# yxyxcyx/Real-Time-Recommendation-System-with-Feature-Store

Measured on NVIDIA B200. Metric: top-100 exact-IP QPS over 10M items, higher is better.
Workload: dtype bf16

## Files before the change

real-time-recommendation-system-with-feature-store_b200/csrc/stream_scores.cuh:

```cuda
#pragma once
#include <cstdlib>
#include "host_util.h"
#include "tc_common.cuh"

namespace b200 {

constexpr int ST_EPI_WARP0 = 4;
constexpr int ST_HELP_WARP0 = 12;
constexpr int ST_HELP_WARPS = 4;
constexpr int ST_THREADS = 16 * 32;
constexpr int ST_QTILE_BYTES = 128 * 64 * 2;
constexpr int ST_MAX_STAGES = 16;
constexpr int ST_SMEM_LIMIT = 232448;
constexpr int ST_BAR_BYTES = 512;

struct StreamGeom {
  long long N;
  long long T;
  long long total;
  long long W;
  int Q;
  int KB;
  int S;
  int grid;
// ... 57 lines not shown
__device__ __forceinline__ int geom_first_cta(const StreamGeom& g, int s) { return (int)((s * g.T) / g.W); }
__device__ __forceinline__ int geom_last_cta(const StreamGeom& g, int s) { return (int)(((s + 1) * g.T - 1) / g.W); }


template <int NQ, int BN, class Epi>
__global__ void __launch_bounds__(ST_THREADS, 1)
stream_scores_kernel(const __grid_constant__ CUtensorMap tmap_q, const __grid_constant__ CUtensorMap tmap_x,
                     const StreamGeom g, const typename Epi::Args ea) {
  constexpr int QPT = NQ >= 2 ? NQ / 2 : 1;
  constexpr int EPI_WARPS = NQ >= 2 ? 8 : 4;
  constexpr int STAGE_BYTES = BN * 128;
  static_assert(NQ <= 2, "helper-warp mailboxes are sized for 256 resident rows");
  static_assert(2 * NQ * BN <= 512, "two accumulator buffers must fit the 512 TMEM columns");

  extern __shared__ uint8_t smem_raw[];
  uint8_t* smem = smem_raw + ((1024u - (smem_u32(smem_raw) & 1023u)) & 1023u);
  uint8_t* q_smem = smem;
  uint8_t* ring = smem + NQ * g.KB * ST_QTILE_BYTES;
  uint8_t* tail = ring + g.stages * STAGE_BYTES;
  uint64_t* full_bar = reinterpret_cast<uint64_t*>(tail);
  uint64_t* empty_bar = full_bar + ST_MAX_STAGES;
  uint64_t* acc_full = empty_bar + ST_MAX_STAGES;
  uint64_t* acc_empty = acc_full + 2;
  uint64_t* q_full = acc_empty + 2;
  uint64_t* q_empty = q_full + 1;
  uint32_t* tmem_slot = reinterpret_cast<uint32_t*>(q_empty + 1);
  uint32_t* scratch = reinterpret_cast<uint32_t*>(tail + ST_BAR_BYTES);

  const int warp = threadIdx.x >> 5;
  const int lane = threadIdx.x & 31;

  if (warp == 0 && lane == 0) {
    tma_prefetch_desc(&tmap_q);
    tma_prefetch_desc(&tmap_x);
  }
  if (warp == 1 && lane == 0) {
    for (int s = 0; s < g.stages; ++s) {
      mbar_init(&full_bar[s], 1);
      mbar_init(&empty_bar[s], 1);
    }
    for (int b = 0; b < 2; ++b) {
      mbar_init(&acc_full[b], 1);
      mbar_init(&acc_empty[b], EPI_WARPS);
    }
    mbar_init(q_full, 1);
    mbar_init(q_empty, 1);
    fence_mbar_init();
  }
  if (warp == 2) tmem_alloc(tmem_slot, 512);
  if (warp == 3) Epi::init_scratch(scratch, lane);
  tc_fence_before();
  __syncthreads();
  tc_fence_after();
  const uint32_t tmem_base = *tmem_slot;

  const long long w_begin = (long long)blockIdx.x * g.W;
  long long w_end = w_begin + g.W;
  if (w_end > g.total) w_end = g.total;

  if (warp == 0) {
    {
      const uint64_t pol_q = l2_policy_evict_last();
      uint32_t it = 0, seg = 0;
      for (long long w = w_begin; w < w_end; ++seg) {
        const int s = (int)(w / g.T);
        const long long t0 = w - (long long)s * g.T;
        long long t1 = t0 + (w_end - w);
        if (t1 > g.T) t1 = g.T;
        mbar_wait(q_empty, (seg & 1) ^ 1);
        if (elect_one()) {
          mbar_arrive_expect_tx(q_full, NQ * g.KB * ST_QTILE_BYTES);
          for (int qs = 0; qs < NQ; ++qs)
            for (int kb = 0; kb < g.KB; ++kb)
              tma_load_2d_hint(q_smem + (qs * g.KB + kb) * ST_QTILE_BYTES, &tmap_q, q_full, kb * 64,
                               (s * NQ + qs) * 128, pol_q);
        }
        __syncwarp();
        for (long long t = t0; t < t1; ++t) {
          for (int kb = 0; kb < g.KB; ++kb, ++it) {
            const int st = it % g.stages;
            const uint32_t ph = (it / g.stages) & 1;
            mbar_wait(&empty_bar[st], ph ^ 1);
            if (elect_one()) {
              mbar_arrive_expect_tx(&full_bar[st], STAGE_BYTES);
              tma_load_2d(ring + st * STAGE_BYTES, &tmap_x, &full_bar[st], kb * 64, (int)(t * BN));
            }
            __syncwarp();
          }
        }
        w += t1 - t0;
      }
    }
  } else if (warp == 1) {
    {
      const uint32_t idesc = umma_idesc_bf16(128, BN);
      const uint64_t desc_base = umma_desc_k_sw128(0);
      const uint32_t q_lo = (smem_u32(q_smem) & 0x3FFFFu) >> 4;
      const uint32_t ring_lo = (smem_u32(ring) & 0x3FFFFu) >> 4;
      uint32_t it = 0, seg = 0, tc = 0;
      for (long long w = w_begin; w < w_end; ++seg) {
        const int s = (int)(w / g.T);
        const long long t0 = w - (long long)s * g.T;
        long long t1 = t0 + (w_end - w);
        if (t1 > g.T) t1 = g.T;
        mbar_wait(q_full, seg & 1);
        tc_fence_after();
        for (long long t = t0; t < t1; ++t, ++tc) {
          const uint32_t buf = tc & 1;
          mbar_wait(&acc_empty[buf], ((tc >> 1) & 1) ^ 1);
          tc_fence_after();
          for (int kb = 0; kb < g.KB; ++kb, ++it) {
            const int st = it % g.stages;
            const uint32_t ph = (it / g.stages) & 1;
            mbar_wait(&full_bar[st], ph);
            tc_fence_after();
            if (elect_one()) {
              const uint64_t b_desc = desc_base + (ring_lo + ((st * STAGE_BYTES) >> 4));
#pragma unroll
              for (int qs = 0; qs < NQ; ++qs) {
                const uint64_t a_desc = desc_base + (q_lo + (((qs * g.KB + kb) * ST_QTILE_BYTES) >> 4));
                const uint32_t d_addr = tmem_base + (buf * NQ + qs) * BN;
#pragma unroll
                for (int k = 0; k < 4; ++k) umma_bf16(d_addr, a_desc + 2 * k, b_desc + 2 * k, idesc, (kb | k) != 0);
              }
              umma_commit(&empty_bar[st]);
              if (kb == g.KB - 1) umma_commit(&acc_full[buf]);
            }
            __syncwarp();
          }
        }
        if (elect_one()) umma_commit(q_empty);
        __syncwarp();
        w += t1 - t0;
      }
    }
  } else if (warp >= ST_EPI_WARP0 && warp < ST_EPI_WARP0 + EPI_WARPS) {
    const int ew = warp - ST_EPI_WARP0;
    const int quarter = warp & 3;
    const int half = ew >> 2;
    Epi epi;
    uint32_t tc = 0;
    for (long long w = w_begin; w < w_end;) {
      const int s = (int)(w / g.T);
      const long long t0 = w - (long long)s * g.T;
      long long t1 = t0 + (w_end - w);
      if (t1 > g.T) t1 = g.T;
      const int part = (int)blockIdx.x - geom_first_cta(g, s);
      int qslot[QPT];
      long long qrow[QPT];
#pragma unroll
      for (int a = 0; a < QPT; ++a) {
        qslot[a] = (half * QPT + a) * 128 + quarter * 32 + lane;
        const long long q = (long long)s * (128 * NQ) + qslot[a];
        qrow[a] = q < g.Q ? q : -1;
      }
      epi.template begin_segment<128 * NQ, QPT>(ea, g, s, part, qrow, qslot, lane, scratch);
      for (long long t = t0; t < t1; ++t, ++tc) {
        const uint32_t buf = tc & 1;
        epi.template pre_tile<BN, QPT>(ea, g, qslot, lane, scratch);
        mbar_wait(&acc_full[buf], (tc >> 1) & 1);
        tc_fence_after();
#pragma unroll
        for (int a = 0; a < QPT; ++a) {
          const uint32_t taddr =
              tmem_base + (static_cast<uint32_t>(quarter * 32) << 16) + (buf * NQ + half * QPT + a) * BN;
          epi.template tile<BN>(ea, g, a, taddr, (unsigned long long)t * BN);
        }
        tc_fence_before();
        __syncwarp();
        if (lane == 0) mbar_arrive(&acc_empty[buf]);
      }
      epi.template end_segment<128 * NQ, QPT>(ea, g, s, part, qslot, lane, scratch, (w + (t1 - t0)) >= w_end);
      w += t1 - t0;
    }
    Epi::epilogue_exit(scratch, lane);
  } else if (warp >= ST_HELP_WARP0) {
    Epi::template helper<128 * NQ, EPI_WARPS>(ea, g, warp - ST_HELP_WARP0, lane, scratch);
  }
  tc_fence_before();
  __syncthreads();
  if (warp == 2) {
    tc_fence_after();
    tmem_dealloc(tmem_base, 512);
  }
}

}
```

real-time-recommendation-system-with-feature-store_b200/csrc/stream_scores2.cuh:

```cuda
#pragma once
#include "stream_scores.cuh"

namespace b200 {

__device__ __forceinline__ uint32_t cluster_ctarank() {
  uint32_t r;
  asm volatile("mov.u32 %0, %%cluster_ctarank;" : "=r"(r));
  return r;
}
__device__ __forceinline__ void cluster_sync_all() {
  asm volatile("barrier.cluster.arrive.release.aligned;\n\tbarrier.cluster.wait.acquire.aligned;" ::: "memory");
}
__device__ __forceinline__ uint32_t mapa_u32(uint32_t local, uint32_t rank) {
  uint32_t r;
  asm volatile("mapa.shared::cluster.u32 %0, %1, %2;" : "=r"(r) : "r"(local), "r"(rank));
  return r;
}
__device__ __forceinline__ void mbar_arrive_cluster(uint32_t cluster_addr) {
  asm volatile("mbarrier.arrive.shared::cluster.b64 _, [%0];" ::"r"(cluster_addr) : "memory");
}
__device__ __forceinline__ void tma_load_2d_2sm(void* smem_dst, const CUtensorMap* m, uint32_t bar_cluster_addr, int c0,
                                                int c1) {
  asm volatile(
      "cp.async.bulk.tensor.2d.cta_group::2.shared::cluster.global.mbarrier::complete_tx::bytes [%0], [%1, {%3, %4}], [%2];"
// ... 125 lines not shown
stream_scores2_kernel(const __grid_constant__ CUtensorMap tmap_q, const __grid_constant__ CUtensorMap tmap_x,
                      const StreamGeom g, const typename Epi::Args ea) {
  constexpr int EPI_WARPS = 8;
  constexpr int S2_ROWS = S2Shape<NQ2>::ROWS, S2_QUERIES = S2Shape<NQ2>::QUERIES;
  constexpr int S2_STAGE_BYTES = S2Shape<NQ2>::STAGE_BYTES, UMMA_N = S2Shape<NQ2>::UMMA_N;
  constexpr int COLS = 128;
  constexpr int NSUB = NQ2;
  extern __shared__ uint8_t smem_raw[];
  uint8_t* smem = smem_raw + ((1024u - (smem_u32(smem_raw) & 1023u)) & 1023u);
  uint8_t* q_smem = smem;
  uint8_t* ring = smem + NQ2 * g.KB * ST_QTILE_BYTES;
  const int ks = g.ks;
  const int stage_bytes = S2_STAGE_BYTES * ks;
  const int nsteps = g.KB / ks;
  uint8_t* tail = ring + g.stages * stage_bytes;
  uint64_t* full_bar = reinterpret_cast<uint64_t*>(tail);
  uint64_t* empty_bar = full_bar + ST_MAX_STAGES;
  uint64_t* acc_full = empty_bar + ST_MAX_STAGES;
  uint64_t* acc_empty = acc_full + 4;
  uint64_t* q_full = acc_empty + 4;
  uint64_t* q_empty = q_full + 1;
  uint32_t* tmem_slot = reinterpret_cast<uint32_t*>(q_empty + 1);
  uint32_t* scratch = reinterpret_cast<uint32_t*>(tail + ST_BAR_BYTES);

  const int warp = threadIdx.x >> 5;
  const int lane = threadIdx.x & 31;
  const uint32_t rank = cluster_ctarank();
  const bool leader = rank == 0;
  const long long unit = blockIdx.x >> 1;

  if (warp == 0 && lane == 0) {
    tma_prefetch_desc(&tmap_q);
    tma_prefetch_desc(&tmap_x);
  }
  if (warp == 1 && lane == 0) {
    for (int s = 0; s < g.stages; ++s) {
      mbar_init(&full_bar[s], 1);
      mbar_init(&empty_bar[s], 1);
    }
    for (int b = 0; b < 4; ++b) {
      mbar_init(&acc_full[b], 1);
      mbar_init(&acc_empty[b], 2 * EPI_WARPS / NSUB);
    }
    mbar_init(q_full, 1);
    mbar_init(q_empty, 1);
    fence_mbar_init();
  }
  if (warp == 2) tmem_alloc2(tmem_slot, 512);
  if (warp == 3) Epi::init_scratch(scratch, lane);
  tc_fence_before();
  __syncthreads();
  cluster_sync_all();
  tc_fence_after();
  const uint32_t tmem_base = *tmem_slot;

  constexpr bool kDbg = Epi::kDbg;
  const bool dbg_st = kDbg && (g.dbg_stats == 1 || g.dbg_stats == 2 + (int)unit);
  const bool nofeed = kDbg && g.dbg_nofeed != 0;
  const int mma_order = kDbg ? g.mma_order : 0;
  int s;
  long long t0, ntile, tstep;
  bool last_seg;

  if (warp == 0) {
    {
      const uint32_t q_full_leader = mapa_u32(smem_u32(q_full), 0);
      uint32_t it = 0;
      for (int seg = 0; geom2_segment(g, unit, seg, s, t0, ntile, tstep, last_seg); ++seg) {
        mbar_wait(q_empty, (seg & 1) ^ 1);
        if (elect_one()) {
          if (leader) mbar_arrive_expect_tx(q_full, 2 * NQ2 * g.KB * ST_QTILE_BYTES);
          for (int qt = 0; qt < NQ2; ++qt)
            for (int kb = 0; kb < g.KB; ++kb)
              tma_load_2d_2sm(q_smem + (qt * g.KB + kb) * ST_QTILE_BYTES, &tmap_q, q_full_leader, kb * 64,
                              s * S2_QUERIES + qt * 256 + (int)rank * 128);
        }
        __syncwarp();
        if (!nofeed) {
          for (long long ti = 0, t = t0; ti < ntile; ++ti, t += tstep) {
            for (int step = 0; step < nsteps; ++step, ++it) {
              const int st = it % g.stages;
              const uint32_t ph = (it / g.stages) & 1;
              mbar_wait(&empty_bar[st], ph ^ 1);
              if (elect_one()) {
                if (leader) mbar_arrive_expect_tx(&full_bar[st], 2 * stage_bytes);
                const uint32_t bar = mapa_u32(smem_u32(&full_bar[st]), 0);
                for (int a = 0; a < ks; ++a)
                  tma_load_2d_2sm(ring + st * stage_bytes + a * S2_STAGE_BYTES, &tmap_x, bar, (step * ks + a) * 64,
                                  (int)(t * S2_ROWS + rank * (S2_ROWS / 2)));
              }
              __syncwarp();
            }
          }
        }
      }
    }
  } else if (warp == 1) {
    if (leader) {
      const uint32_t idesc = umma_idesc_bf16(256, UMMA_N);
      const uint64_t desc_base = umma_desc_k_sw128(0);
      const uint32_t q_lo = (smem_u32(q_smem) & 0x3FFFFu) >> 4;
      const uint32_t ring_lo = (smem_u32(ring) & 0x3FFFFu) >> 4;
      uint32_t it = 0, tc = 0;
      long long c_acc = 0, c_full = 0;
      for (int seg = 0; geom2_segment(g, unit, seg, s, t0, ntile, tstep, last_seg); ++seg) {
        mbar_wait(q_full, seg & 1);
// ... 44 lines not shown
          tc_fence_after();
          const long long c1 = dbg_st ? clock64() : 0;
          c_acc += c1 - c0;
          for (int step = 0; step < nsteps; ++step, ++it) {
            const int st = it % g.stages;
            const uint32_t ph = (it / g.stages) & 1;
            if (!nofeed) {
              const long long c2 = dbg_st ? clock64() : 0;
              mbar_wait(&full_bar[st], ph);
              tc_fence_after();
              if (dbg_st) c_full += clock64() - c2;
            }
            if (elect_one()) {
              for (int a = 0; a < ks; ++a) {
                const int kb = step * ks + a;
                const uint64_t b_desc = desc_base + (ring_lo + ((st * stage_bytes + a * S2_STAGE_BYTES) >> 4));
                if (mma_order == 3) {
#pragma unroll
                  for (int k = 0; k < 4; ++k) {
#pragma unroll
                    for (int qt = 0; qt < NQ2; ++qt) {
                      const uint64_t a_desc = desc_base + (q_lo + (((qt * g.KB + kb) * ST_QTILE_BYTES) >> 4));
                      umma_bf16_2sm(tmem_base + buf * 256 + qt * 128, a_desc + 2 * k, b_desc + 2 * k, idesc, (kb | k) != 0);
                    }
                  }
                  continue;
                }
#pragma unroll
                for (int qt = 0; qt < NQ2; ++qt) {
                  const uint64_t a_desc = desc_base + (q_lo + (((qt * g.KB + kb) * ST_QTILE_BYTES) >> 4));
                  const uint32_t d_addr = tmem_base + buf * 256 + qt * 128;
#pragma unroll
                  for (int k = 0; k < 4; ++k)
                    umma_bf16_2sm(d_addr, a_desc + 2 * k, b_desc + 2 * k, idesc, (kb | k) != 0);
                }
              }
              if (!nofeed) umma_commit_2sm(&empty_bar[st]);
              if (step == nsteps - 1) {
                for (int sub = 0; sub < NSUB; ++sub) umma_commit_2sm(&acc_full[buf * 2 + sub]);
              }
            }
            __syncwarp();
          }
        }
        if (elect_one()) umma_commit_2sm(q_empty);
        __syncwarp();
      }
      if (dbg_st && lane == 0) {
        atomicAdd(&g_stream_stats[0], (unsigned long long)c_acc);
        atomicAdd(&g_stream_stats[1], (unsigned long long)c_full);
      }
    }
  } else if (warp >= ST_EPI_WARP0 && warp < ST_EPI_WARP0 + EPI_WARPS) {
    const int ew = warp - ST_EPI_WARP0;
    const int quarter = warp & 3;
    const int half = ew >> 2;
    Epi epi;
    uint32_t tc = 0;
    long long c_wait = 0, c_proc = 0;
    const int sub = NSUB == 2 ? half : 0;
    const uint32_t acc_empty_leader[2] = {mapa_u32(smem_u32(&acc_empty[sub]), 0), mapa_u32(smem_u32(&acc_empty[2 + sub]), 0)};
    for (int seg = 0; geom2_segment(g, unit, seg, s, t0, ntile, tstep, last_seg); ++seg) {
      const int part = 0;
      int qslot[1] = {half * 128 + quarter * 32 + lane};
      const long long q = (long long)s * S2_QUERIES + (NQ2 == 2 ? half * 256 : 0) + rank * 128 + quarter * 32 + lane;
      long long qrow[1] = {q < g.Q ? q : -1};
      epi.template begin_segment<S2_SLOTS, 1>(ea, g, s, part, qrow, qslot, lane, scratch);
      for (long long ti = 0, t = t0; ti < ntile; ++ti, t += tstep, ++tc) {
        const uint32_t buf = tc & 1;
        epi.template pre_tile<COLS, 1>(ea, g, qslot, lane, scratch);
        const long long c0 = dbg_st ? clock64() : 0;
        mbar_wait(&acc_full[buf * 2 + sub], (tc >> 1) & 1);
        tc_fence_after();
        const long long c1 = dbg_st ? clock64() : 0;
        const uint32_t taddr = tmem_base + (static_cast<uint32_t>(quarter * 32) << 16) + buf * 256 + half * 128;
        epi.template tile<COLS>(ea, g, 0, taddr, (unsigned long long)t * S2_ROWS + (NQ2 == 1 ? half * 128 : 0));
        tc_fence_before();
        __syncwarp();
        if (lane == 0) mbar_arrive_cluster(acc_empty_leader[buf]);
        if (dbg_st) {
          c_wait += c1 - c0;
          c_proc += clock64() - c1;
        }
      }
      epi.template end_segment<S2_SLOTS, 1>(ea, g, s, part, qslot, lane, scratch, last_seg);
    }
    if (dbg_st && lane == 0) {
      atomicAdd(&g_stream_stats[2], (unsigned long long)c_wait);
      atomicAdd(&g_stream_stats[3], (unsigned long long)c_proc);
      atomicAdd(&g_stream_stats[4], (unsigned long long)tc);
    }
    Epi::epilogue_exit(scratch, lane);
  } else if (warp >= ST_HELP_WARP0) {
    Epi::template helper<S2_SLOTS, EPI_WARPS>(ea, g, warp - ST_HELP_WARP0, lane, scratch);
  }
  tc_fence_before();
  __syncthreads();
  cluster_sync_all();
  if (warp == 2) {
    tc_fence_after();
    tmem_dealloc2(tmem_base, 512);
  }
}

}
```

real-time-recommendation-system-with-feature-store_b200/csrc/tc_common.cuh:

```cuda
#pragma once
#include <cuda.h>
#include <cuda_runtime.h>
#include <cuda_bf16.h>
#include <stdint.h>

namespace b200 {

constexpr uint32_t FULL_MASK = 0xffffffffu;

__device__ __forceinline__ uint32_t smem_u32(const void* p) {
  return static_cast<uint32_t>(__cvta_generic_to_shared(p));
}
__device__ __forceinline__ bool elect_one() {
  uint32_t pred;
  asm volatile(
      "{\n\t.reg .pred p;\n\t"
      "elect.sync _|p, 0xffffffff;\n\t"
      "selp.u32 %0, 1, 0, p;\n\t}\n"
      : "=r"(pred));
  return pred != 0;
}

__device__ __forceinline__ void mbar_init(uint64_t* bar, uint32_t count) {
  asm volatile("mbarrier.init.shared::cta.b64 [%0], %1;" ::"r"(smem_u32(bar)), "r"(count) : "memory");
}
__device__ __forceinline__ void fence_mbar_init() {
  asm volatile("fence.mbarrier_init.release.cluster;" ::: "memory");
}
__device__ __forceinline__ void fence_proxy_async_smem() {
  asm volatile("fence.proxy.async.shared::cta;" ::: "memory");
}
__device__ __forceinline__ void mbar_arrive(uint64_t* bar) {
  asm volatile("mbarrier.arrive.shared::cta.b64 _, [%0];" ::"r"(smem_u32(bar)) : "memory");
}
__device__ __forceinline__ void mbar_arrive_expect_tx(uint64_t* bar, uint32_t bytes) {
  asm volatile("mbarrier.arrive.expect_tx.shared::cta.b64 _, [%0], %1;" ::"r"(smem_u32(bar)), "r"(bytes)
               : "memory");
}
__device__ __forceinline__ bool mbar_try_wait(uint64_t* bar, uint32_t parity) {
  uint32_t ok;
  asm volatile(
      "{\n\t.reg .pred p;\n\t"
      "mbarrier.try_wait.parity.shared::cta.b64 p, [%1], %2;\n\t"
      "selp.u32 %0, 1, 0, p;\n\t}\n"
      : "=r"(ok)
      : "r"(smem_u32(bar)), "r"(parity)
      : "memory");
  return ok != 0;
}
__device__ __forceinline__ void mbar_wait(uint64_t* bar, uint32_t parity) {
  uint32_t spins = 0;
  while (!mbar_try_wait(bar, parity)) {
    if (++spins > (1u << 24)) {
      printf("b200rec: mbarrier wait timed out (block %d thread %d)\n", blockIdx.x, threadIdx.x);
      __trap();
    }
  }
}

__device__ __forceinline__ void tma_prefetch_desc(const CUtensorMap* m) {
  asm volatile("prefetch.tensormap [%0];" ::"l"(reinterpret_cast<uint64_t>(m)) : "memory");
}
__device__ __forceinline__ void tma_load_2d(void* smem_dst, const CUtensorMap* m, uint64_t* bar, int c0, int c1) {
  asm volatile(
      "cp.async.bulk.tensor.2d.shared::cluster.global.mbarrier::complete_tx::bytes [%0], [%1, {%3, %4}], [%2];"
      ::"r"(smem_u32(smem_dst)), "l"(reinterpret_cast<uint64_t>(m)), "r"(smem_u32(bar)), "r"(c0), "r"(c1)
      : "memory");
}
__device__ __forceinline__ void tma_load_2d_hint(void* smem_dst, const CUtensorMap* m, uint64_t* bar, int c0,
                                                  int c1, uint64_t policy) {
  asm volatile(
      "cp.async.bulk.tensor.2d.shared::cluster.global.mbarrier::complete_tx::bytes.L2::cache_hint"
      " [%0], [%1, {%3, %4}], [%2], %5;"
      ::"r"(smem_u32(smem_dst)), "l"(reinterpret_cast<uint64_t>(m)), "r"(smem_u32(bar)), "r"(c0), "r"(c1),
      "l"(policy)
      : "memory");
}
__device__ __forceinline__ uint64_t l2_policy_evict_first() {
  uint64_t p;
  asm volatile("createpolicy.fractional.L2::evict_first.b64 %0, 1.0;" : "=l"(p));
  return p;
// ... 120 lines not shown
```

real-time-recommendation-system-with-feature-store_b200/csrc/topk.cu:

```cuda
#include <cfloat>
#include <cstdlib>
#include <mutex>
#include "stream_scores.cuh"
#include "stream_scores2.cuh"
#include "../../include/b200rec.h"

namespace b200 {

__device__ __forceinline__ int warp_pick_digit(const uint32_t* hist, int& need, int& bucket, int lane) {
  uint32_t c[8];
  uint32_t lane_total = 0;
#pragma unroll
  for (int b = 0; b < 8; ++b) {
    c[b] = hist[lane * 8 + b];
    lane_total += c[b];
  }
  uint32_t incl = lane_total;
#pragma unroll
  for (int o = 1; o < 32; o <<= 1) {
    const uint32_t t = __shfl_down_sync(FULL_MASK, incl, o);
    if (lane + o < 32) incl += t;
  }
  const uint32_t above = incl - lane_total;
  const bool mine = (above < (uint32_t)need) && ((uint32_t)need <= incl);
// ... 520 lines not shown
          __syncwarp();
          if (lane == 0) {
            __threadfence();
            atomicExch(&m->lock, 0u);
            reqs[slot] = 0u;
          }
          __syncwarp();
          if (dbgv(ea) == 2 && lane == 0) atomicAdd(&g_topk_stats[3], (unsigned long long)(clock64() - hb0));
        }
      }
      if (!any) {
        if (finished) break;
        __nanosleep(ea.hsleep);
      }
    }
    if (stamp) {
      unsigned long long ns_end;
      asm volatile("mov.u64 %0, %%globaltimer;" : "=l"(ns_end));
      if (blockIdx.x == 0) g_topk_stats[6] = (unsigned long long)(clock64() - c_begin) * 1000ull / (ns_end - ns_begin + 1);
      atomicMax(&g_topk_stats[5], ~ns_begin);
      atomicMax(&g_topk_stats[7], ns_end);
      if (blockIdx.x < 512) g_cta_end[blockIdx.x] = ns_end;
    }
  }
};

using TopkEpi = TopkEpiT<false>;
using TopkEpiDbg = TopkEpiT<true>;

struct SampleMaxEpi {
  static constexpr bool kDbg = false;
  static constexpr int SCRATCH_BYTES = 64;
  struct Args {
    float* out;
    int ngroups;
    int gw;
  };
  long long qrow[2];

  static __device__ __forceinline__ void init_scratch(uint32_t*, int) {}
  static __device__ __forceinline__ void epilogue_exit(uint32_t*, int) {}
  template <int SLOTS, int EPI_WARPS>
  static __device__ __forceinline__ void helper(const Args&, const StreamGeom&, int, int, uint32_t*) {}

  template <int SLOTS, int QPT>
  __device__ __forceinline__ void begin_segment(const Args&, const StreamGeom&, int, int, const long long (&q)[QPT],
                                                const int (&)[QPT], int, uint32_t*) {
#pragma unroll
    for (int a = 0; a < QPT; ++a) qrow[a] = q[a];
  }
  template <int BN, int QPT>
  __device__ __forceinline__ void pre_tile(const Args&, const StreamGeom&, const int (&)[QPT], int, uint32_t*) {}

  template <int BN>
  __device__ __forceinline__ void tile(const Args& ea, const StreamGeom&, int a, uint32_t taddr,
                                       unsigned long long row0) {
    float run = -INFINITY;
#pragma unroll 1
    for (int c = 0; c < BN; c += 32) {
      uint32_t v[32];
      tmem_ld_32x32(taddr + c, v);
      tmem_ld_wait();
      float m4[4];
#pragma unroll
      for (int j = 0; j < 4; ++j) {
        const float m0 = fmax3(__uint_as_float(v[8 * j + 0]), __uint_as_float(v[8 * j + 1]), __uint_as_float(v[8 * j + 2]));
        const float m1 = fmax3(__uint_as_float(v[8 * j + 3]), __uint_as_float(v[8 * j + 4]), __uint_as_float(v[8 * j + 5]));
        m4[j] = fmax3(m0, m1, fmaxf(__uint_as_float(v[8 * j + 6]), __uint_as_float(v[8 * j + 7])));
      }
      run = fmaxf(run, fmaxf(fmaxf(m4[0], m4[1]), fmaxf(m4[2], m4[3])));
      if (((c + 32) % ea.gw) == 0) {
        if (qrow[a] >= 0) ea.out[(size_t)qrow[a] * ea.ngroups + (row0 + c) / ea.gw] = run;
        run = -INFINITY;
      }
    }
  }

  template <int SLOTS, int QPT>
  __device__ __forceinline__ void end_segment(const Args&, const StreamGeom&, int, int, const int (&)[QPT], int,
                                              uint32_t*, bool) {}
};

constexpr int FIN_THREADS = 256;

template <class Loader>
__device__ void block_select_sort_core(const Loader& load, int n, int k_out, uint64_t* skeys , int P,
                                       uint32_t* hist , int* s_misc ) {
  const int tid = threadIdx.x, lane = tid & 31, warp = tid >> 5;
  if (tid == 0) s_misc[0] = 0;
  __syncthreads();
  int local = 0;
  for (int i = tid; i < n; i += FIN_THREADS) local += load(i) != 0ull;
  for (int o = 16; o > 0; o >>= 1) local += __shfl_xor_sync(FULL_MASK, local, o);
  if (lane == 0 && local) atomicAdd(&s_misc[0], local);
  __syncthreads();
  const int n_valid = s_misc[0];
  uint64_t prefix = 1;
  int shift = 0;
  if (n_valid > k_out) {
    prefix = 0;
    shift = 56;
    int need = k_out;
    for (int pass = 0; pass < 8; ++pass, shift -= 8) {
      hist[tid] = 0;
      __syncthreads();
      for (int i = tid; i < n; i += FIN_THREADS) {
        const uint64_t key = load(i);
        const bool match = (pass == 0) || ((key >> (shift + 8)) == prefix);
        if (match && key != 0ull) atomicAdd(&hist[(uint32_t)(key >> shift) & 255u], 1u);
      }
      __syncthreads();
      if (warp == 0) {
        int bucket;
        const int d = warp_pick_digit(hist, need, bucket, lane);
        if (lane == 0) {
          s_misc[1] = d;
          s_misc[2] = need;
          s_misc[3] = bucket;
        }
      }
      __syncthreads();
      prefix = (prefix << 8) | (uint64_t)s_misc[1];
      need = s_misc[2];
      const int bucket = s_misc[3];
      __syncthreads();
      if (bucket == need) break;
// ... 46 lines not shown

constexpr int FAN_MAX = 16;
struct OutFan {
  int n;
  float* s[FAN_MAX];
  int64_t* i[FAN_MAX];
};

__device__ __forceinline__ void write_result(const uint64_t* skeys, int k_out, int64_t row_offset, float* out_s,
                                             int64_t* out_i) {
  for (int i = threadIdx.x; i < k_out; i += FIN_THREADS) {
    const uint64_t key = skeys[i];
    if (key == 0ull) {
      out_s[i] = -FLT_MAX;
      out_i[i] = -1;
    } else {
      out_s[i] = ord_f32((uint32_t)(key >> 32));
      out_i[i] = (int64_t)(~(uint32_t)key) + row_offset;
    }
  }
}

constexpr int FIN_MAX_SRC = 160;
struct MultiLoader {
  const uint64_t* const* ptr;
  const int* off;
  int nsrc;
  __device__ __forceinline__ uint64_t operator()(int i) const {
    int lo = 0, hi = nsrc - 1;
    while (lo < hi) {
      const int mid = (lo + hi + 1) >> 1;
      if (off[mid] <= i)
        lo = mid;
      else
        hi = mid - 1;
    }
    return __ldcg(ptr[lo] + (i - off[lo]));
  }
};

__global__ void __launch_bounds__(FIN_THREADS)
topk_final_kernel(const StreamGeom g, int v2, int qs , int slots ,
                  const uint64_t* __restrict__ tlists, const QMeta* __restrict__ meta,
                  const uint64_t* __restrict__ lists, const uint32_t* __restrict__ left, int cap, int k, int P,
                  int stage_cap, int64_t row_offset, const OutFan fan) {
  extern __shared__ uint64_t fin_smem[];
  __shared__ uint32_t hist[256];
  __shared__ int s_misc[8];
  __shared__ const uint64_t* s_ptr[FIN_MAX_SRC];
  __shared__ int s_off[FIN_MAX_SRC + 1];
  __shared__ int s_last[FIN_MAX_SRC];
  const int q = blockIdx.x;
  const int s = q / qs, inq = q - s * qs;
  if (v2) {
    for (int u = threadIdx.x; u < g.grid / 2 && u < FIN_MAX_SRC; u += FIN_THREADS) s_last[u] = geom2_last_super(g, u);
    __syncthreads();
  }
  if (threadIdx.x == 0) {
    int n = 0, ns = 0;
    s_ptr[ns] = tlists + (size_t)q * 2 * k + (size_t)meta[q].tsel * k;
    s_off[ns++] = n;
    n += (int)meta[q].tcount;
    const int u0 = v2 ? 0 : geom_first_cta(g, s), u1 = v2 ? g.grid / 2 - 1 : geom_last_cta(g, s);
    for (int u = u0; u <= u1; ++u) {
      if (v2) {
        if (u >= FIN_MAX_SRC || s_last[u] != s) continue;
      } else {
        long long wend = (long long)(u + 1) * g.W;
        if (wend > g.total) wend = g.total;
        if ((int)((wend - 1) / g.T) != s) continue;
      }
      const int cta = v2 ? 2 * u + ((inq >> 7) & 1) : u;
      const int nslot = v2 == 1 ? 2 : 1;
      for (int h = 0; h < nslot && ns < FIN_MAX_SRC; ++h) {
        const int slot = v2 == 1 ? h * 128 + (inq & 127) : (v2 == 2 ? (inq >> 8) * 128 + (inq & 127) : inq);
        const uint32_t l = left[(size_t)cta * slots + slot];
        const int cnt = (int)(l & 0x7FFFFFFFu);
        if (cnt == 0) continue;
        s_ptr[ns] = lists + ((size_t)cta * slots + slot) * (2 * (size_t)cap) + ((l >> 31) ? cap : 0);
        s_off[ns++] = n;
        n += cnt;
      }
    }
    s_off[ns] = n;
    s_misc[5] = ns;
    s_misc[6] = n;
  }
  __syncthreads();
  MultiLoader ld{s_ptr, s_off, s_misc[5]};
  const int n = s_misc[6];
  __syncthreads();
  block_select_sort(ld, n, k, fin_smem, P, hist, s_misc, fin_smem + P, stage_cap);
  for (int d = 0; d < fan.n; ++d)
    write_result(fin_smem, k, row_offset, fan.s[d] + (size_t)q * k, fan.i[d] + (size_t)q * k);
}

struct FloatRowLoader {
  const float* row;
  __device__ __forceinline__ uint64_t operator()(int i) const {
    return (static_cast<uint64_t>(f32_ord(__ldcg(row + i))) << 32) | static_cast<uint64_t>(~(uint32_t)i);
  }
};
__global__ void __launch_bounds__(FIN_THREADS)
sample_topk_kernel(const float* __restrict__ S, int m, int k, int P, int stage_cap, const OutFan fan) {
  extern __shared__ uint64_t fin_smem[];
  __shared__ uint32_t hist[256];
  __shared__ int s_misc[8];
  const int q = blockIdx.x;
  FloatRowLoader ld{S + (size_t)q * m};
  block_select_sort(ld, m, k, fin_smem, P, hist, s_misc, fin_smem + P, stage_cap);
  for (int i = threadIdx.x; i < k; i += FIN_THREADS) {
    const uint64_t key = fin_smem[i];
    const float v = key == 0ull ? -FLT_MAX : ord_f32((uint32_t)(key >> 32));
    for (int d = 0; d < fan.n; ++d) fan.s[d][(size_t)q * k + i] = v;
  }
}

struct PooledLoader {
  const float* vals;
  size_t part_stride;
  int k_in;
  __device__ __forceinline__ uint64_t operator()(int i) const {
    const int p = i / k_in, j = i - p * k_in;
    return (static_cast<uint64_t>(f32_ord(__ldcg(vals + (size_t)p * part_stride + j))) << 32) | static_cast<uint64_t>(~(uint32_t)i);
  }
};
__global__ void __launch_bounds__(FIN_THREADS)
pooled_kth_kernel(const float* __restrict__ vals, int parts, long long Q, int k_in, int k, int P, int stage_cap,
                  float* __restrict__ out_kth) {
  extern __shared__ uint64_t fin_smem[];
  __shared__ uint32_t hist[256];
  __shared__ int s_misc[8];
  const long long q = blockIdx.x;
  PooledLoader ld{vals + (size_t)q * k_in, (size_t)Q * k_in, k_in};
  block_select_sort(ld, parts * k_in, k, fin_smem, P, hist, s_misc, fin_smem + P, stage_cap);
  if (threadIdx.x == 0) {
    const uint64_t key = fin_smem[k - 1];
    out_kth[q] = key == 0ull ? -FLT_MAX : ord_f32((uint32_t)(key >> 32));
  }
}

__global__ void topk_init_from_kernel(QMeta* meta, int Q, const float* __restrict__ tau_init) {
  const int q = blockIdx.x * blockDim.x + threadIdx.x;
  if (q < Q) {
    uint32_t key = f32_ord(tau_init[q]);
    key = key > 64u ? key - 64u : 0u;
    QMeta m;
    m.lock = 0u;
    m.tcount = 0u;
    m.tsel = 0u;
    m.tau = fmaxf(ord_f32(key), nextafterf(-FLT_MAX, 0.f));
    meta[q] = m;
  }
}

__global__ void topk_init_kernel(QMeta* meta, int Q, float tau0) {
  const int q = blockIdx.x * blockDim.x + threadIdx.x;
  if (q < Q) {
    QMeta m;
    m.lock = 0u;
    m.tcount = 0u;
    m.tsel = 0u;
    m.tau = tau0;
    meta[q] = m;
  }
}

struct ListLoader {
  const float* scores;
  const int64_t* ids;
  size_t s_stride, i_stride;
  int k_in;
  __device__ __forceinline__ uint64_t operator()(int i) const {
    const int p = i / k_in, j = i - p * k_in;
    const int64_t id = ids[(size_t)p * i_stride + j];
    return id < 0 ? 0ull : make_key(scores[(size_t)p * s_stride + j], (uint32_t)id);
  }
};

__global__ void __launch_bounds__(FIN_THREADS)
topk_merge_kernel(const float* __restrict__ scores, const int64_t* __restrict__ ids, int parts, long long Q, int k_in,
                  int k_out, int P, int stage_cap, long long s_stride, long long i_stride,
                  float* __restrict__ out_scores, int64_t* __restrict__ out_ids) {
  extern __shared__ uint64_t fin_smem[];
  __shared__ uint32_t hist[256];
  __shared__ int s_misc[8];
  const long long q = blockIdx.x;
  ListLoader ld;
  ld.scores = scores + (size_t)q * k_in;
  ld.ids = ids + (size_t)q * k_in;
  ld.s_stride = (size_t)s_stride;
  ld.i_stride = (size_t)i_stride;
  ld.k_in = k_in;
  block_select_sort(ld, parts * k_in, k_out, fin_smem, P, hist, s_misc, fin_smem + P, stage_cap);
  write_result(fin_smem, k_out, 0, out_scores + (size_t)q * k_out, out_ids + (size_t)q * k_out);
}

__global__ void __launch_bounds__(FIN_THREADS)
sample_kth_kernel(const float* __restrict__ S, int m, int k, QMeta* __restrict__ meta) {
  __shared__ uint32_t hist[256];
  __shared__ int s_misc[4];
  const int q = blockIdx.x, tid = threadIdx.x, lane = tid & 31, warp = tid >> 5;
  const float* row = S + (size_t)q * m;
  uint32_t prefix = 0;
  int need = k, shift = 24;
  for (int pass = 0; pass < 4; ++pass, shift -= 8) {
    hist[tid] = 0;
    __syncthreads();
    for (int i = tid; i < m; i += FIN_THREADS) {
      const uint32_t key = f32_ord(__ldcg(row + i));
      const bool match = (pass == 0) || ((key >> (shift + 8)) == prefix);
      if (match) atomicAdd(&hist[(key >> shift) & 255u], 1u);
    }
    __syncthreads();
    if (warp == 0) {
      int bucket, nd = need;
      const int d = warp_pick_digit(hist, nd, bucket, lane);
      if (lane == 0) {
        s_misc[0] = d;
        s_misc[1] = nd;
        s_misc[2] = bucket;
      }
    }
    __syncthreads();
    prefix = (prefix << 8) | (uint32_t)s_misc[0];
    need = s_misc[1];
    const int bucket = s_misc[2];
    __syncthreads();
    if (bucket == need) break;
  }
  if (shift < 0) shift = 0;
  if (tid == 0) {
    uint32_t key = prefix << shift;
    key = key > 64u ? key - 64u : 0u;
    const float floor0 = nextafterf(-FLT_MAX, 0.f);
    QMeta mm;
    mm.lock = 0u;
    mm.tcount = 0u;
    mm.tsel = 0u;
    mm.tau = fmaxf(ord_f32(key), floor0);
    meta[q] = mm;
  }
}

static int next_pow2(int v) {
  int p = 1;
  while (p < v) p <<= 1;
  return p;
}

static int g_time_kernel = 0;
static cudaEvent_t g_ev0 = nullptr, g_ev1 = nullptr;

struct TopkPlan {
  int v2;
  int nq, bn;
  StreamGeom g;
  int cap;
  size_t lists_bytes, tlists_bytes, meta_bytes, left_bytes, sample_bytes;
  int64_t sample_m, sample_stride;
  int sample_gw;
  int sample_k_out;
  StreamGeom gs;
  size_t total() const { return lists_bytes + tlists_bytes + meta_bytes + left_bytes + sample_bytes; }
};
// ... 101 lines not shown
  p.sample_gw = 32;
  const int64_t n_pool = N * (shards > 1 ? shards : 1);
  int64_t frac = n_pool >= (4ll << 20) ? 32 : (n_pool >= (256ll << 10) ? 16 : 8);
  if (shards > 1 && frac > 8) frac /= 2;
  if (kn.sample_frac > 0) frac = kn.sample_frac;
  int64_t m = (N / frac) / 256 * 256;
  if (!kn.nosample && m >= 2048) {
    int gw = 32;
    while (gw < 128 && gw < p.bn && m / gw > 8192) gw *= 2;
    if (m / gw >= 2 * (int64_t)k) {
      p.sample_m = m;
      p.sample_stride = N / m;
      p.sample_gw = gw;
      p.sample_bytes = (size_t)Q * (m / gw) * sizeof(float);
      bool sok;
      if (p.v2 == 2) sok = stream_geom2<2>(p.gs, m, (int)Q, KB, sms, SampleMaxEpi::SCRATCH_BYTES);
      else if (p.v2 == 1) sok = stream_geom2<1>(p.gs, m, (int)Q, KB, sms, SampleMaxEpi::SCRATCH_BYTES);
      else if (p.nq == 2) sok = stream_geom<2, 128>(p.gs, m, (int)Q, KB, sms, SampleMaxEpi::SCRATCH_BYTES);
      else if (p.bn == 256) sok = stream_geom<1, 256>(p.gs, m, (int)Q, KB, sms, SampleMaxEpi::SCRATCH_BYTES);
      else sok = stream_geom<1, 64>(p.gs, m, (int)Q, KB, sms, SampleMaxEpi::SCRATCH_BYTES);
      if (!sok) p.sample_m = 0, p.sample_bytes = 0;
    }
  }
  return 0;
}

struct PlanKey {
  int64_t N, ld, Q;
  int k, shards;
  bool operator==(const PlanKey& o) const { return N == o.N && ld == o.ld && Q == o.Q && k == o.k && shards == o.shards; }
};
static PlanKey g_plan_keys[64];
static TopkPlan g_plans[64];
static int g_plan_used = 0, g_plan_next = 0;

static int plan_topk(TopkPlan& p, int64_t N, int64_t ld, int64_t Q, int k, int shards = 1) {
  const PlanKey key{N, ld, Q, k, shards};
  {
    std::lock_guard<std::mutex> lock(g_cache_mu);
    for (int i = 0; i < g_plan_used; ++i)
      if (g_plan_keys[i] == key) {
        p = g_plans[i];
        return 0;
      }
  }
  if (plan_topk_uncached(p, N, ld, Q, k, shards)) return 1;
  std::lock_guard<std::mutex> lock(g_cache_mu);
  const int slot = g_plan_used < 64 ? g_plan_used++ : (g_plan_next = (g_plan_next + 1) % 64);
  g_plan_keys[slot] = key;
  g_plans[slot] = p;
  return 0;
}

template <int NQ, int BN, int V2, bool DBG>
static int launch_topk(const TopkPlan& p, const void* catalogue, int64_t N, int64_t ld, const void* queries, int64_t Q,
                       int k, int64_t row_offset, const int64_t* excl_indptr, const int32_t* excl_rows,
                       float* out_scores, int64_t* out_ids, void* workspace, cudaStream_t st,
                       const float* tau_init, float* sample_vals_out, const OutFan* fan_in) {
  OutFan fan;
  if (fan_in != nullptr) {
    fan = *fan_in;
  } else {
    fan.n = 1;
    fan.s[0] = sample_vals_out != nullptr ? sample_vals_out : out_scores;
    fan.i[0] = out_ids;
  }
  using Epi = TopkEpiT<DBG>;
  const TopkKnobs& kn = knobs();
  CUtensorMap tq, tx;
  if (cached_tmap(&tq, queries, (uint64_t)Q, (uint64_t)ld, (uint64_t)ld, 128)) return 1;
  constexpr int XBOX = V2 == 1 ? 128 : (V2 == 2 ? 64 : BN);
  if (cached_tmap(&tx, catalogue, (uint64_t)N, (uint64_t)ld, (uint64_t)ld, XBOX)) return 1;
  TopkArgs ea;
  ea.lists = reinterpret_cast<uint64_t*>(workspace);
  ea.tlists = reinterpret_cast<uint64_t*>(reinterpret_cast<uint8_t*>(workspace) + p.lists_bytes);
  ea.meta = reinterpret_cast<QMeta*>(reinterpret_cast<uint8_t*>(workspace) + p.lists_bytes + p.tlists_bytes);
  ea.left = reinterpret_cast<uint32_t*>(reinterpret_cast<uint8_t*>(workspace) + p.lists_bytes + p.tlists_bytes + p.meta_bytes);
  B200_CUDA_OK(cudaMemsetAsync(ea.left, 0, p.left_bytes, st));
  ea.excl_indptr = excl_indptr;
  ea.excl_rows = excl_rows;
  ea.k = k;
  ea.cap = p.cap;
  ea.flush = kn.flush >= 0 ? kn.flush : ((k > 128 && Q <= 256) ? p.cap : (k / 4 > 32 ? (k / 4) / 32 * 32 : 32));
  ea.debug = kn.debug;
  ea.hsleep = kn.hsleep;
  void (*kern)(const CUtensorMap, const CUtensorMap, const StreamGeom, const TopkArgs);
  if constexpr (V2 != 0) kern = stream_scores2_kernel<(V2 == 2 ? 2 : 1), Epi>;
  else kern = stream_scores_kernel<NQ, BN, Epi>;
  static int smem_set = 0;
  if (smem_set < p.g.smem_bytes) {
    B200_CUDA_OK(cudaFuncSetAttribute(kern, cudaFuncAttributeMaxDynamicSharedMemorySize, ST_SMEM_LIMIT));
    smem_set = ST_SMEM_LIMIT;
  }
  if (tau_init != nullptr) {
    topk_init_from_kernel<<<(unsigned)((Q + 255) / 256), 256, 0, st>>>(ea.meta, (int)Q, tau_init);
    B200_LAUNCH_OK("topk_init_from_kernel");
  } else if (p.sample_m > 0 && excl_indptr == nullptr) {
    float* S = reinterpret_cast<float*>(reinterpret_cast<uint8_t*>(workspace) + p.lists_bytes + p.tlists_bytes + p.meta_bytes + p.left_bytes);
    CUtensorMap ts;
    if (cached_tmap(&ts, catalogue, (uint64_t)p.sample_m, (uint64_t)ld, (uint64_t)(ld * p.sample_stride), XBOX)) return 1;
    SampleMaxEpi::Args sa;
    sa.out = S;
    sa.ngroups = (int)(p.sample_m / p.sample_gw);
    sa.gw = p.sample_gw;
    void (*skern)(const CUtensorMap, const CUtensorMap, const StreamGeom, const SampleMaxEpi::Args);
    if constexpr (V2 != 0) skern = stream_scores2_kernel<(V2 == 2 ? 2 : 1), SampleMaxEpi>;
    else skern = stream_scores_kernel<NQ, BN, SampleMaxEpi>;
    static bool sattr = false;
    if (!sattr) {
      B200_CUDA_OK(cudaFuncSetAttribute(skern, cudaFuncAttributeMaxDynamicSharedMemorySize, ST_SMEM_LIMIT));
      sattr = true;
    }
    skern<<<p.gs.grid, ST_THREADS, p.gs.smem_bytes, st>>>(tq, ts, p.gs, sa);
    B200_LAUNCH_OK("stream_scores_kernel<sample>");
    if (sample_vals_out != nullptr) {
      const int P = next_pow2(k);
      const int sc = sa.ngroups <= 4096 ? sa.ngroups : 0;
      sample_topk_kernel<<<(unsigned)Q, FIN_THREADS, (P + sc) * sizeof(uint64_t), st>>>(S, sa.ngroups, p.sample_k_out, P, sc, fan);
      B200_LAUNCH_OK("sample_topk_kernel");
      return 0;
    }
    sample_kth_kernel<<<(unsigned)Q, FIN_THREADS, 0, st>>>(S, sa.ngroups, k, ea.meta);
    B200_LAUNCH_OK("sample_kth_kernel");
  } else if (sample_vals_out != nullptr) {
    return fail("topk_sample: no sampling pass for this shape (catalogue too small or exclusion lists given)");
  } else {
    topk_init_kernel<<<(unsigned)((Q + 255) / 256), 256, 0, st>>>(ea.meta, (int)Q, nextafterf(-FLT_MAX, 0.f));
    B200_LAUNCH_OK("topk_init_kernel");
  }
  if (g_time_kernel) {
    if (!g_ev0) {
      B200_CUDA_OK(cudaEventCreate(&g_ev0));
      B200_CUDA_OK(cudaEventCreate(&g_ev1));
    }
    B200_CUDA_OK(cudaEventRecord(g_ev0, st));
  }
  StreamGeom gl = p.g;
  gl.dbg_nofeed = (ea.debug == 4) ? 1 : 0;
  gl.dbg_stats = (ea.debug == 2 || kn.stream_stats) ? 1 : 0;
  if (kn.stats_unit >= 0) gl.dbg_stats = 2 + kn.stats_unit;
  if (ea.debug == 4) ea.debug = 3;
  kern<<<gl.grid, ST_THREADS, gl.smem_bytes, st>>>(tq, tx, gl, ea);
  B200_LAUNCH_OK("stream_scores_kernel<topk>");
  if (g_time_kernel) B200_CUDA_OK(cudaEventRecord(g_ev1, st));
  const int P = next_pow2(k);
  const int fin_stage = P <= 1024 ? 1024 : 0;
  topk_final_kernel<<<(unsigned)Q, FIN_THREADS, (P + fin_stage) * sizeof(uint64_t), st>>>(
      p.g, V2, V2 == 2 ? 512 : (V2 == 1 ? 256 : 128 * NQ), V2 ? S2_SLOTS : 128 * NQ, ea.tlists, ea.meta, ea.lists, ea.left, p.cap,
      k, P, fin_stage, row_offset, fan);
  B200_LAUNCH_OK("topk_final_kernel");
  return 0;
}

}

extern "C" int b200rec_debug_reload_env(void) {
  using namespace b200;
  std::lock_guard<std::mutex> lock(g_cache_mu);
  knobs() = read_knobs();
  stream_knobs() = read_stream_knobs();
  g_plan_used = g_plan_next = 0;
  return 0;
}

extern "C" int b200rec_debug_topk_stats(unsigned long long* out8_host, int reset) {
  using namespace b200;
  B200_CUDA_OK(cudaMemcpyFromSymbol(out8_host, g_topk_stats, sizeof(unsigned long long) * 8));
  if (reset) {
    unsigned long long z[8] = {0};
    B200_CUDA_OK(cudaMemcpyToSymbol(g_topk_stats, z, sizeof(z)));
  }
  return 0;
}

extern "C" int b200rec_debug_topk_stats16(unsigned long long* out24_host, int reset) {
  using namespace b200;
  B200_CUDA_OK(cudaMemcpyFromSymbol(out24_host, g_topk_stats, sizeof(unsigned long long) * 16));
  B200_CUDA_OK(cudaMemcpyFromSymbol(out24_host + 16, g_stream_stats, sizeof(unsigned long long) * 8));
  if (reset) {
    unsigned long long z[16] = {0};
    B200_CUDA_OK(cudaMemcpyToSymbol(g_topk_stats, z, sizeof(z)));
    B200_CUDA_OK(cudaMemcpyToSymbol(g_stream_stats, z, sizeof(unsigned long long) * 8));
  }
  return 0;
}

extern "C" int b200rec_debug_topk_cta_end(unsigned long long* out512_host) {
  using namespace b200;
  B200_CUDA_OK(cudaMemcpyFromSymbol(out512_host, g_cta_end, sizeof(unsigned long long) * 512));
  return 0;
}

extern "C" int b200rec_debug_topk_kernel_timing(int enable, float* last_ms_host) {
  using namespace b200;
  if (last_ms_host) {
    *last_ms_host = 0.f;
    if (g_ev0 && g_ev1) {
      B200_CUDA_OK(cudaEventSynchronize(g_ev1));
      B200_CUDA_OK(cudaEventElapsedTime(last_ms_host, g_ev0, g_ev1));
    }
  }
  g_time_kernel = enable;
// ... 133 lines not shown
```

Before: 465,300.

## Add programmatic dependent launch, vectorize sample-max epilogue, stage kth-select keys

Launches the stream-scoring and final top-k kernels with programmatic stream serialization. Prologues (barrier init, TMEM alloc) now overlap the previous kernel's tail, and consumer warps wait on griddepcontrol before reading upstream results. The sample-max epilogue batches two TMEM loads per wait and writes group maxima with vector stores. sample_kth stages keys in shared memory and uses warp match_any to aggregate histogram atomics. It also drops the memset of the per-query 'left' counters, which risks stale state unless something else resets them.

```diff
diff --git a/real-time-recommendation-system-with-feature-store_b200/csrc/stream_scores.cuh b/real-time-recommendation-system-with-feature-store_b200/csrc/stream_scores.cuh
--- a/real-time-recommendation-system-with-feature-store_b200/csrc/stream_scores.cuh
+++ b/real-time-recommendation-system-with-feature-store_b200/csrc/stream_scores.cuh
@@ -133,6 +133,7 @@
   tc_fence_before();
   __syncthreads();
   tc_fence_after();
+  griddep_launch_dependents();
   const uint32_t tmem_base = *tmem_slot;
 
   const long long w_begin = (long long)blockIdx.x * g.W;
@@ -216,6 +217,7 @@
       }
     }
   } else if (warp >= ST_EPI_WARP0 && warp < ST_EPI_WARP0 + EPI_WARPS) {
+    griddep_wait();
     const int ew = warp - ST_EPI_WARP0;
     const int quarter = warp & 3;
     const int half = ew >> 2;
@@ -256,6 +258,7 @@
     }
     Epi::epilogue_exit(scratch, lane);
   } else if (warp >= ST_HELP_WARP0) {
+    griddep_wait();
     Epi::template helper<128 * NQ, EPI_WARPS>(ea, g, warp - ST_HELP_WARP0, lane, scratch);
   }
   tc_fence_before();
diff --git a/real-time-recommendation-system-with-feature-store_b200/csrc/stream_scores2.cuh b/real-time-recommendation-system-with-feature-store_b200/csrc/stream_scores2.cuh
--- a/real-time-recommendation-system-with-feature-store_b200/csrc/stream_scores2.cuh
+++ b/real-time-recommendation-system-with-feature-store_b200/csrc/stream_scores2.cuh
@@ -201,6 +201,7 @@
   __syncthreads();
   cluster_sync_all();
   tc_fence_after();
+  griddep_launch_dependents();
   const uint32_t tmem_base = *tmem_slot;
 
   constexpr bool kDbg = Epi::kDbg;
@@ -351,6 +352,7 @@
       }
     }
   } else if (warp >= ST_EPI_WARP0 && warp < ST_EPI_WARP0 + EPI_WARPS) {
+    griddep_wait();
     const int ew = warp - ST_EPI_WARP0;
     const int quarter = warp & 3;
     const int half = ew >> 2;
@@ -391,6 +393,7 @@
     }
     Epi::epilogue_exit(scratch, lane);
   } else if (warp >= ST_HELP_WARP0) {
+    griddep_wait();
     Epi::template helper<S2_SLOTS, EPI_WARPS>(ea, g, warp - ST_HELP_WARP0, lane, scratch);
   }
   tc_fence_before();
diff --git a/real-time-recommendation-system-with-feature-store_b200/csrc/tc_common.cuh b/real-time-recommendation-system-with-feature-store_b200/csrc/tc_common.cuh
--- a/real-time-recommendation-system-with-feature-store_b200/csrc/tc_common.cuh
+++ b/real-time-recommendation-system-with-feature-store_b200/csrc/tc_common.cuh
@@ -27,6 +27,8 @@
 __device__ __forceinline__ void fence_mbar_init() {
   asm volatile("fence.mbarrier_init.release.cluster;" ::: "memory");
 }
+__device__ __forceinline__ void griddep_wait() { asm volatile("griddepcontrol.wait;" ::: "memory"); }
+__device__ __forceinline__ void griddep_launch_dependents() { asm volatile("griddepcontrol.launch_dependents;" ::: "memory"); }
 __device__ __forceinline__ void fence_proxy_async_smem() {
   asm volatile("fence.proxy.async.shared::cta;" ::: "memory");
 }
diff --git a/real-time-recommendation-system-with-feature-store_b200/csrc/topk.cu b/real-time-recommendation-system-with-feature-store_b200/csrc/topk.cu
--- a/real-time-recommendation-system-with-feature-store_b200/csrc/topk.cu
+++ b/real-time-recommendation-system-with-feature-store_b200/csrc/topk.cu
@@ -596,26 +596,57 @@
   template <int BN, int QPT>
   __device__ __forceinline__ void pre_tile(const Args&, const StreamGeom&, const int (&)[QPT], int, uint32_t*) {}
 
+  static __device__ __forceinline__ float max32(const uint32_t (&v)[32]) {
+    float m4[4];
+#pragma unroll
+    for (int j = 0; j < 4; ++j) {
+      const float m0 = fmax3(__uint_as_float(v[8 * j + 0]), __uint_as_float(v[8 * j + 1]), __uint_as_float(v[8 * j + 2]));
+      const float m1 = fmax3(__uint_as_float(v[8 * j + 3]), __uint_as_float(v[8 * j + 4]), __uint_as_float(v[8 * j + 5]));
+      m4[j] = fmax3(m0, m1, fmaxf(__uint_as_float(v[8 * j + 6]), __uint_as_float(v[8 * j + 7])));
+    }
+    return fmaxf(fmaxf(m4[0], m4[1]), fmaxf(m4[2], m4[3]));
+  }
+  template <int NB, int G>
+  static __device__ __forceinline__ void store_groups(float* dst, const float (&m32)[NB]) {
+    constexpr int PER = NB / G;
+    float gm[G];
+#pragma unroll
+    for (int j = 0; j < G; ++j) {
+      float run = -INFINITY;
+#pragma unroll
+      for (int i = 0; i < PER; ++i) run = fmaxf(run, m32[j * PER + i]);
+      gm[j] = run;
+    }
+    if constexpr (G == 4) *reinterpret_cast<float4*>(dst) = make_float4(gm[0], gm[1], gm[2], gm[3]);
+    else if constexpr (G == 2) *reinterpret_cast<float2*>(dst) = make_float2(gm[0], gm[1]);
+    else dst[0] = gm[0];
+  }
+
   template <int BN>
   __device__ __forceinline__ void tile(const Args& ea, const StreamGeom&, int a, uint32_t taddr,
                                        unsigned long long row0) {
-    float run = -INFINITY;
+    constexpr int CH = BN < 128 ? BN : 128;
+    constexpr int NB = CH / 32;
 #pragma unroll 1
-    for (int c = 0; c < BN; c += 32) {
-      uint32_t v[32];
-      tmem_ld_32x32(taddr + c, v);
-      tmem_ld_wait();
-      float m4[4];
-#pragma unroll
-      for (int j = 0; j < 4; ++j) {
-        const float m0 = fmax3(__uint_as_float(v[8 * j + 0]), __uint_as_float(v[8 * j + 1]), __uint_as_float(v[8 * j + 2]));
-        const float m1 = fmax3(__uint_as_float(v[8 * j + 3]), __uint_as_float(v[8 * j + 4]), __uint_as_float(v[8 * j + 5]));
-        m4[j] = fmax3(m0, m1, fmaxf(__uint_as_float(v[8 * j + 6]), __uint_as_float(v[8 * j + 7])));
-      }
-      run = fmaxf(run, fmaxf(fmaxf(m4[0], m4[1]), fmaxf(m4[2], m4[3])));
-      if (((c + 32) % ea.gw) == 0) {
-        if (qrow[a] >= 0) ea.out[(size_t)qrow[a] * ea.ngroups + (row0 + c) / ea.gw] = run;
-        run = -INFINITY;
+    for (int c0 = 0; c0 < BN; c0 += CH) {
+      float m32[NB];
+#pragma unroll
+      for (int c = 0; c < CH; c += 64) {
+        uint32_t v0[32], v1[32];
+        tmem_ld_32x32(taddr + c0 + c, v0);
+        tmem_ld_32x32(taddr + c0 + c + 32, v1);
+        tmem_ld_wait();
+        m32[c / 32] = max32(v0);
+        m32[c / 32 + 1] = max32(v1);
+      }
+      if (qrow[a] < 0) continue;
+      float* dst = ea.out + (size_t)qrow[a] * ea.ngroups + (row0 + c0) / ea.gw;
+      if (ea.gw == 32) {
+        store_groups<NB, NB>(dst, m32);
+      } else if (ea.gw == 64) {
+        store_groups<NB, NB / 2>(dst, m32);
+      } else if constexpr (NB >= 4) {
+        store_groups<NB, NB / 4>(dst, m32);
       }
     }
   }
@@ -768,6 +799,7 @@
   __shared__ int s_last[FIN_MAX_SRC];
   const int q = blockIdx.x;
   const int s = q / qs, inq = q - s * qs;
+  griddep_wait();
   if (v2) {
     for (int u = threadIdx.x; u < g.grid / 2 && u < FIN_MAX_SRC; u += FIN_THREADS) s_last[u] = geom2_last_super(g, u);
     __syncthreads();
@@ -857,6 +889,7 @@
 }
 
 __global__ void topk_init_from_kernel(QMeta* meta, int Q, const float* __restrict__ tau_init) {
+  griddep_launch_dependents();
   const int q = blockIdx.x * blockDim.x + threadIdx.x;
   if (q < Q) {
     uint32_t key = f32_ord(tau_init[q]);
@@ -871,6 +904,7 @@
 }
 
 __global__ void topk_init_kernel(QMeta* meta, int Q, float tau0) {
+  griddep_launch_dependents();
   const int q = blockIdx.x * blockDim.x + threadIdx.x;
   if (q < Q) {
     QMeta m;
@@ -912,21 +946,31 @@
   write_result(fin_smem, k_out, 0, out_scores + (size_t)q * k_out, out_ids + (size_t)q * k_out);
 }
 
+constexpr int SAMPLE_KTH_STAGE = 8192;
 __global__ void __launch_bounds__(FIN_THREADS)
-sample_kth_kernel(const float* __restrict__ S, int m, int k, QMeta* __restrict__ meta) {
+sample_kth_kernel(const float* __restrict__ S, int m, int k, QMeta* __restrict__ meta, int staged) {
+  extern __shared__ uint32_t kth_keys[];
   __shared__ uint32_t hist[256];
   __shared__ int s_misc[4];
   const int q = blockIdx.x, tid = threadIdx.x, lane = tid & 31, warp = tid >> 5;
+  griddep_launch_dependents();
   const float* row = S + (size_t)q * m;
+  if (staged) {
+    for (int i = tid; i < m; i += FIN_THREADS) kth_keys[i] = f32_ord(__ldcg(row + i));
+  }
+  const int m_pad = (m + FIN_THREADS - 1) / FIN_THREADS * FIN_THREADS;
   uint32_t prefix = 0;
   int need = k, shift = 24;
   for (int pass = 0; pass < 4; ++pass, shift -= 8) {
     hist[tid] = 0;
     __syncthreads();
-    for (int i = tid; i < m; i += FIN_THREADS) {
-      const uint32_t key = f32_ord(__ldcg(row + i));
-      const bool match = (pass == 0) || ((key >> (shift + 8)) == prefix);
-      if (match) atomicAdd(&hist[(key >> shift) & 255u], 1u);
+    for (int i = tid; i < m_pad; i += FIN_THREADS) {
+      uint32_t key = 0u;
+      if (i < m) key = staged ? kth_keys[i] : f32_ord(__ldcg(row + i));
+      const bool match = (i < m) && ((pass == 0) || ((key >> (shift + 8)) == prefix));
+      const uint32_t bin = match ? ((key >> shift) & 255u) : 256u;
+      const uint32_t peers = __match_any_sync(FULL_MASK, bin);
+      if (match && (__ffs(peers) - 1) == lane) atomicAdd(&hist[bin], (uint32_t)__popc(peers));
     }
     __syncthreads();
     if (warp == 0) {
@@ -1134,6 +1178,22 @@
   return 0;
 }
 
+template <class... KArgs, class... Args>
+static cudaError_t launch_after_prev(void (*kern)(KArgs...), dim3 grid, dim3 block, size_t smem, cudaStream_t st,
+                                     Args... args) {
+  cudaLaunchConfig_t cfg = {};
+  cfg.gridDim = grid;
+  cfg.blockDim = block;
+  cfg.dynamicSmemBytes = smem;
+  cfg.stream = st;
+  cudaLaunchAttribute attr[1];
+  attr[0].id = cudaLaunchAttributeProgrammaticStreamSerialization;
+  attr[0].val.programmaticStreamSerializationAllowed = 1;
+  cfg.attrs = attr;
+  cfg.numAttrs = 1;
+  return cudaLaunchKernelEx(&cfg, kern, static_cast<KArgs>(args)...);
+}
+
 template <int NQ, int BN, int V2, bool DBG>
 static int launch_topk(const TopkPlan& p, const void* catalogue, int64_t N, int64_t ld, const void* queries, int64_t Q,
                        int k, int64_t row_offset, const int64_t* excl_indptr, const int32_t* excl_rows,
@@ -1158,7 +1218,6 @@
   ea.tlists = reinterpret_cast<uint64_t*>(reinterpret_cast<uint8_t*>(workspace) + p.lists_bytes);
   ea.meta = reinterpret_cast<QMeta*>(reinterpret_cast<uint8_t*>(workspace) + p.lists_bytes + p.tlists_bytes);
   ea.left = reinterpret_cast<uint32_t*>(reinterpret_cast<uint8_t*>(workspace) + p.lists_bytes + p.tlists_bytes + p.meta_bytes);
-  B200_CUDA_OK(cudaMemsetAsync(ea.left, 0, p.left_bytes, st));
   ea.excl_indptr = excl_indptr;
   ea.excl_rows = excl_rows;
   ea.k = k;
@@ -1202,7 +1261,9 @@
       B200_LAUNCH_OK("sample_topk_kernel");
       return 0;
     }
-    sample_kth_kernel<<<(unsigned)Q, FIN_THREADS, 0, st>>>(S, sa.ngroups, k, ea.meta);
+    const int kth_staged = sa.ngroups <= SAMPLE_KTH_STAGE ? 1 : 0;
+    sample_kth_kernel<<<(unsigned)Q, FIN_THREADS, kth_staged ? sa.ngroups * sizeof(uint32_t) : 0, st>>>(S, sa.ngroups, k,
+                                                                                                        ea.meta, kth_staged);
     B200_LAUNCH_OK("sample_kth_kernel");
   } else if (sample_vals_out != nullptr) {
     return fail("topk_sample: no sampling pass for this shape (catalogue too small or exclusion lists given)");
@@ -1222,14 +1283,14 @@
   gl.dbg_stats = (ea.debug == 2 || kn.stream_stats) ? 1 : 0;
   if (kn.stats_unit >= 0) gl.dbg_stats = 2 + kn.stats_unit;
   if (ea.debug == 4) ea.debug = 3;
-  kern<<<gl.grid, ST_THREADS, gl.smem_bytes, st>>>(tq, tx, gl, ea);
+  B200_CUDA_OK(launch_after_prev(kern, dim3(gl.grid), dim3(ST_THREADS), gl.smem_bytes, st, tq, tx, gl, ea));
   B200_LAUNCH_OK("stream_scores_kernel<topk>");
   if (g_time_kernel) B200_CUDA_OK(cudaEventRecord(g_ev1, st));
   const int P = next_pow2(k);
   const int fin_stage = P <= 1024 ? 1024 : 0;
-  topk_final_kernel<<<(unsigned)Q, FIN_THREADS, (P + fin_stage) * sizeof(uint64_t), st>>>(
-      p.g, V2, V2 == 2 ? 512 : (V2 == 1 ? 256 : 128 * NQ), V2 ? S2_SLOTS : 128 * NQ, ea.tlists, ea.meta, ea.lists, ea.left, p.cap,
-      k, P, fin_stage, row_offset, fan);
+  B200_CUDA_OK(launch_after_prev(topk_final_kernel, dim3((unsigned)Q), dim3(FIN_THREADS), (P + fin_stage) * sizeof(uint64_t), st,
+      p.g, (int)V2, V2 == 2 ? 512 : (V2 == 1 ? 256 : 128 * NQ), V2 ? S2_SLOTS : 128 * NQ, (const uint64_t*)ea.tlists,
+      (const QMeta*)ea.meta, (const uint64_t*)ea.lists, (const uint32_t*)ea.left, p.cap, k, P, fin_stage, row_offset, fan));
   B200_LAUNCH_OK("topk_final_kernel");
   return 0;
 }
```

Result: no change. 463,700 (median of 6 runs) (-0.3%).
